# lms-org/trajectory_controller

Hardware: AMD Instinct MI355X
Metric: MPC QP solves/sec (horizon N=20, 2 inputs) at 1/2/4/8 MI355X; max|du| vs dlib (higher is better)
Workload: dtype f64; 1 GPU; batch 262144 trajectories per GPU, N=20, 2 inputs, compact (mpcControllerTobi) form, cold start, eps 0.01, max_iter 10000; global_batch=262144, horizon=20, algo=lane_fma, parallelism=batch-sharded x1, batches_in_flight=1, gather=none (1 GPU)

## Files before the change

trajectory_controller_amd/csrc/mpc_internal.h:

```cpp
#pragma once

#include <hip/hip_runtime.h>
#include <stdint.h>

namespace tpc {

constexpr int kWave = 64;

struct Knobs {
    double eps;
    uint32_t max_iter;
    uint32_t smo_iters;
};

struct CompactArgs {
    int64_t n;
    const void *v, *dy, *dphi;
    void *front, *rear;
    int32_t* iters;
    uint32_t* flags;
    const int32_t* work_hint;
    double step, wheelbase;
    double q[2], r[2], lo[2], hi[2];
    int table_key;
// ... 7 lines not shown
    double q[2], r[2], lo[2], hi[2];
    uint64_t* out;
    uint64_t* info;
    static constexpr int32_t* iters = nullptr;
    static constexpr uint32_t* flags = nullptr;
};

struct GeneralArgs {
    int64_t n, ld;
    const void *A, *B, *C, *Q, *R, *lo, *hi, *x0, *targets;
    void *controls, *v;
    void* u0;
    int32_t* iters;
    uint32_t* flags;
    const int32_t* work_hint;
    int shift_controls;
};

struct Workspace {
    void* state;
    uint32_t* ticket;
    unsigned long long* stats;
    int64_t capacity_bytes;
    uint32_t *keys, *rank, *order;
    void* sort_temp;
    size_t sort_temp_bytes;
    hipEvent_t* ev;
    int wave_group = 0;
    int group_lanes = 0;
    int max_waves = 0;
    bool group_pair = false;
    int64_t lanex_below = -1;
    int cu_count = 0;
};

constexpr int kQueueTickets = 16;
constexpr int kQueueTicketStride = 64;
constexpr int64_t kQueueTicketBytes = (int64_t)kQueueTickets * kQueueTicketStride * 4;
constexpr int64_t kWaveQueueMaxInstances = 32768;

constexpr int kAlgoMixed = 101;
constexpr int kAlgoGeneric = 100;
constexpr int kMaxHorizon = 64;
int64_t generic_scratch_bytes(int H, int dtype, int64_t n);
hipError_t generic_compact(int dtype, int H, const CompactArgs& a, const Knobs& k, void* scratch, hipStream_t s);
hipError_t generic_general(int dtype, int I, int H, const GeneralArgs& a, const Knobs& k, void* scratch, hipStream_t s);

size_t sort_temp_bytes(int64_t n);
hipError_t order_begin(void* temp, hipStream_t s);
hipError_t presolve_merge(const uint32_t* queue, const uint32_t* queue_len, int64_t n, const void* sf, const void* sr,
                          const int32_t* si, void* f, void* r, int32_t* it, uint32_t limit, hipStream_t s);
hipError_t presolve_merge_rows(const uint32_t* queue, const uint32_t* queue_len, int64_t n, const void* su, const int32_t* si,
                               void* u, int32_t* it, int rows, int64_t ld, uint32_t limit, hipStream_t s);
const uint32_t* order_queue_len(const void* temp);
hipError_t order_finish(const uint32_t* keys, const uint32_t* rank, uint32_t* order, int64_t n, void* temp,
                        hipStream_t s);

struct RolloutStepArgs {
    int64_t n, ld, ld_out, ld_nlt;
    int I, H, step, steps;
    const void *A, *B, *C;
    void* x;
    void* targets;
    const void* controls;
    const void* new_last_targets;
    void* controls_out;
    void* states_out;
    const int32_t* iters_step;
    int32_t* iters_out;
    void* sequences_out;
    const void* disturbance;
    int64_t ld_d;
};
hipError_t launch_rollout_step(int dtype, const RolloutStepArgs& a, hipStream_t s);

struct FollowArgs {
    int64_t n, ld;
    int max_points;
    const float *px, *py, *dx, *dy, *vel;
    const int32_t* count;
// ... 23 lines not shown
```

trajectory_controller_amd/csrc/mpc_lane_inst.hip:

```cpp
#include <cstdint>

#include "mpc_lane.h"
#include "mpc_lanex.h"

#ifndef TPC_LANE_H
#error "compile with -DTPC_LANE_H=<horizon>"
#endif

namespace tpc {

namespace {

constexpr int kH = TPC_LANE_H;

template <class Tag, class Kernel>
inline int pg_grid(Kernel kernel, int block) {
    constexpr int kMaxDev = 64;
    static int cache[kMaxDev] = {0};
    int dev = 0;
    if (hipGetDevice(&dev) != hipSuccess) dev = 0;
    if (dev >= 0 && dev < kMaxDev && cache[dev] > 0) return cache[dev];
    int cus = 256, per_cu = 4;
    hipDeviceProp_t prop;
    if (hipGetDeviceProperties(&prop, dev) == hipSuccess) cus = prop.multiProcessorCount;
    if (hipOccupancyMaxActiveBlocksPerMultiprocessor(&per_cu, kernel, block, 0) != hipSuccess || per_cu < 1)
        per_cu = 1;
    if (per_cu > 4) per_cu = 4;
    if (dev >= 0 && dev < kMaxDev) cache[dev] = cus * per_cu;
    return cus * per_cu;
}
struct TagState {}; struct TagFast {}; struct TagExact {}; struct TagLanex {}; template <int I> struct TagLanexG {};

inline bool wants_state(const CompactArgs&) { return false; }
inline bool wants_state(const GeneralArgs& a) { return a.controls != nullptr || a.v != nullptr; }

template <typename T, int I, class Model, class Args>
hipError_t phase1(const Args& a, const Knobs& k, const Workspace& ws, hipStream_t s) {
    T* recs = (T*)ws.state;
    hipError_t e = hipMemsetAsync(ws.ticket, 0, sizeof(uint32_t), s);
    if (e == hipSuccess) e = hipMemsetAsync(ws.stats, 0, 3 * sizeof(unsigned long long), s);
    if (e == hipSuccess) e = order_begin(ws.sort_temp, s);
    if (e != hipSuccess) return e;
    const int cd_grid = (int)((a.n + kWave - 1) / kWave);
    if (ws.ev) (void)hipEventRecord(ws.ev[0], s);
    hipLaunchKernelGGL((lane_cd_kernel<T, I, kH, Model, Args>), dim3(cd_grid), dim3(kWave), 0, s, a, k, recs,
                       ws.keys, ws.rank, (uint32_t*)ws.sort_temp, ws.stats, wants_state(a) ? 0 : 1);
    e = hipGetLastError();
    if (e != hipSuccess) return e;
    e = order_finish(ws.keys, ws.rank, ws.order, a.n, ws.sort_temp, s);
    if (e != hipSuccess) return e;
    if (ws.ev) (void)hipEventRecord(ws.ev[1], s);
    return hipSuccess;
}
template <typename T, int I, class Model, class Args>
hipError_t phase2(const Args& a, const Knobs& k, const Workspace& ws, hipStream_t s, bool only_if_refused) {
    T* recs = (T*)ws.state;
    if (wants_state(a)) {
        const int grid_cap = pg_grid<TagState>(lane_pg_kernel<T, I, kH, Model, Args>, kWave);
        const int64_t need = (a.n + kWave - 1) / kWave;
        hipLaunchKernelGGL((lane_pg_kernel<T, I, kH, Model, Args>), dim3((unsigned)(need < grid_cap ? need : grid_cap)),
                           dim3(kWave), 0, s, a, k, (const T*)recs, (const uint32_t*)ws.order, ws.ticket, ws.stats,
                           only_if_refused ? 1 : 0);
    } else {
        constexpr int bt = kWave * FusedOcc<T, kH>::value;
        const int64_t need = (a.n + bt - 1) / bt;
        const uint32_t* queue_len = order_queue_len(ws.sort_temp);
        if constexpr (Model::kFastStop) {
            if (!only_if_refused) {
                const int fast_cap = pg_grid<TagFast>(lane_pg_fused_kernel<T, I, kH, Model, Args, true>, bt);
                hipLaunchKernelGGL((lane_pg_fused_kernel<T, I, kH, Model, Args, true>),
                                   dim3((unsigned)(need < fast_cap ? need : fast_cap)), dim3(bt), 0, s, a, k,
                                   (const T*)recs, (const uint32_t*)ws.order, ws.ticket, ws.stats, queue_len);
            }
        }
// ... 32 lines not shown
        }
    }
    if constexpr (std::is_same<Args, GeneralArgs>::value && sizeof(T) == 8 && LanexPlan<kH>::built) {
        if (a.n < lanex_below(ws, true)) {
            constexpr int ng = LanexPlan<kH>::NG;
            const int64_t need = (a.n + ng - 1) / ng;
            if (wants_state(a)) {
                const int grid_cap = pg_grid<TagLanexG<I + 2>>(lanexg_pg_kernel<T, I, kH, true>, kWave);
                hipLaunchKernelGGL((lanexg_pg_kernel<T, I, kH, true>), dim3((unsigned)(need < grid_cap ? need : grid_cap)), dim3(kWave), 0, s,
                                   a, k, (const T*)ws.state, (const uint32_t*)ws.order, ws.ticket, ws.stats, (const uint32_t*)nullptr,
                                   GroupRefillBatch<LanexPlan<kH>::G>::value);
            } else {
                const int grid_cap = pg_grid<TagLanexG<I>>(lanexg_pg_kernel<T, I, kH>, kWave);
                hipLaunchKernelGGL((lanexg_pg_kernel<T, I, kH>), dim3((unsigned)(need < grid_cap ? need : grid_cap)), dim3(kWave), 0, s, a, k,
                                   (const T*)ws.state, (const uint32_t*)ws.order, ws.ticket, ws.stats, order_queue_len(ws.sort_temp),
                                   GroupRefillBatch<LanexPlan<kH>::G>::value);
            }
            e = hipGetLastError();
            if (ws.ev) (void)hipEventRecord(ws.ev[2], s);
            return e;
        }
    }
    e = phase2<T, I, Model, Args>(a, k, ws, s, false);
    if (ws.ev) (void)hipEventRecord(ws.ev[2], s);
    return e;
}

template <typename T, int I, class Model, class Args, int SUBSET = 1>
hipError_t resolve(const Args& a, const Knobs& k, const Workspace& ws, const int32_t* select, const uint32_t* gate, hipStream_t s,
                   double lambda_from = 0.0, const uint32_t* pre_len = nullptr, uint32_t pre_limit = 0u) {
    if (a.n <= 0) return hipSuccess;
    T* recs = (T*)ws.state;
    uint32_t* queue_len = ws.ticket + 1;
    hipError_t e = hipMemsetAsync(ws.ticket, 0, 32, s);
    if (e != hipSuccess) return e;
    const int grid = (int)((a.n + kWave - 1) / kWave);
    hipLaunchKernelGGL((lane_cd_kernel<T, I, kH, Model, Args, SUBSET>), dim3(grid), dim3(kWave), 0, s, a, k, recs, ws.order,
                       (uint32_t*)nullptr, queue_len, ws.stats, 1, select, gate, (T)lambda_from, pre_len, pre_limit);
    if constexpr (std::is_same<Model, CompactModel<T>>::value && sizeof(T) == 8 && LanexPlan<kH>::built) {
        constexpr int ng = LanexPlan<kH>::NG;
        const int64_t need = (a.n + ng - 1) / ng;
        if constexpr (SUBSET == 2) {
            const int64_t solo = (int64_t)pre_limit / ng;
            hipLaunchKernelGGL((lanex_pg_kernel<T, kH, true>), dim3((unsigned)(need < solo ? need : solo)), dim3(kWave), 0, s, a, k,
                               (const T*)recs, (const uint32_t*)ws.order, ws.ticket, ws.stats, (const uint32_t*)queue_len, 1, pre_limit);
            return hipGetLastError();
        }
        const int grid_cap = pg_grid<TagLanex>(lanex_pg_kernel<T, kH>, kWave);
        hipLaunchKernelGGL((lanex_pg_kernel<T, kH>), dim3((unsigned)(need < grid_cap ? need : grid_cap)), dim3(kWave), 0, s, a, k,
                           (const T*)recs, (const uint32_t*)ws.order, ws.ticket, ws.stats, (const uint32_t*)queue_len, 1);
        return hipGetLastError();
    } else if constexpr (std::is_same<Args, GeneralArgs>::value && sizeof(T) == 8 && LanexPlan<kH>::built) {
        constexpr int ng = LanexPlan<kH>::NG;
        const int64_t need = (a.n + ng - 1) / ng;
        if constexpr (SUBSET == 2) {
            const int64_t solo = (int64_t)pre_limit / ng;
            hipLaunchKernelGGL((lanexg_pg_kernel<T, I, kH, false, true>), dim3((unsigned)(need < solo ? need : solo)), dim3(kWave), 0, s,
                               a, k, (const T*)recs, (const uint32_t*)ws.order, ws.ticket, ws.stats, (const uint32_t*)queue_len, 1, pre_limit);
            return hipGetLastError();
        }
        const int grid_cap = pg_grid<TagLanexG<I>>(lanexg_pg_kernel<T, I, kH>, kWave);
        hipLaunchKernelGGL((lanexg_pg_kernel<T, I, kH>), dim3((unsigned)(need < grid_cap ? need : grid_cap)), dim3(kWave), 0, s, a, k,
                           (const T*)recs, (const uint32_t*)ws.order, ws.ticket, ws.stats, (const uint32_t*)queue_len, 1);
        return hipGetLastError();
    } else {
    constexpr int bt = kWave * FusedOcc<T, kH>::value;
    const int64_t need = (a.n + bt - 1) / bt;
// ... 71 lines not shown
```

trajectory_controller_amd/csrc/mpc_sort.hip:

```cpp
#include "mpc_internal.h"

namespace tpc {

namespace {

constexpr int kBins = 1 << 16;

constexpr int kScanBlocks = 64, kScanThreads = 256, kPerThread = kBins / kScanBlocks / kScanThreads;

__global__ __launch_bounds__(kScanThreads) void scan_sums_kernel(const uint32_t* __restrict__ hist,
                                                                 uint32_t* __restrict__ block_sum) {
    __shared__ uint32_t part[kScanThreads / 64];
    const int t = threadIdx.x;
    const int top = kBins - 1 - (blockIdx.x * kScanThreads + t) * kPerThread;
    uint32_t sum = 0;
    for (int j = 0; j < kPerThread; ++j) sum += hist[top - j];
    for (int off = 32; off > 0; off >>= 1) sum += __shfl_down(sum, off);
    if ((t & 63) == 0) part[t >> 6] = sum;
    __syncthreads();
    if (t == 0) {
        uint32_t tot = 0;
        for (int w = 0; w < kScanThreads / 64; ++w) tot += part[w];
        block_sum[blockIdx.x] = tot;
    }
}

__global__ __launch_bounds__(kScanThreads) void scan_apply_kernel(uint32_t* __restrict__ hist,
                                                                  const uint32_t* __restrict__ block_sum) {
    __shared__ uint32_t part[kScanThreads];
    const int t = threadIdx.x;
    const int top = kBins - 1 - (blockIdx.x * kScanThreads + t) * kPerThread;
    uint32_t c[kPerThread], sum = 0;
    for (int j = 0; j < kPerThread; ++j) { c[j] = hist[top - j]; sum += c[j]; }
    part[t] = sum;
    __syncthreads();
    for (int off = 1; off < kScanThreads; off <<= 1) {
        const uint32_t add = t >= off ? part[t - off] : 0u;
        __syncthreads();
        part[t] += add;
        __syncthreads();
    }
    uint32_t base = part[t] - sum;
    for (int b = 0; b < (int)blockIdx.x; ++b) base += block_sum[b];
    for (int j = 0; j < kPerThread; ++j) {
        hist[top - j] = base;
        base += c[j];
    }
}

__global__ void scatter_kernel(const uint32_t* __restrict__ keys, const uint32_t* __restrict__ rank,
                               const uint32_t* __restrict__ base, uint32_t* __restrict__ order, int64_t n) {
    for (int64_t i = (int64_t)blockIdx.x * blockDim.x + threadIdx.x; i < n; i += (int64_t)gridDim.x * blockDim.x)
        order[base[keys[i] >> 16] + rank[i]] = (uint32_t)i;
}

}

size_t sort_temp_bytes(int64_t) { return (size_t)(kBins + kScanBlocks) * sizeof(uint32_t); }

const uint32_t* order_queue_len(const void* temp) { return (const uint32_t*)temp + 127; }

hipError_t order_begin(void* temp, hipStream_t s) {
    return hipMemsetAsync(temp, 0, (size_t)kBins * sizeof(uint32_t), s);
}

hipError_t order_finish(const uint32_t* keys, const uint32_t* rank, uint32_t* order, int64_t n, void* temp,
                        hipStream_t s) {
    uint32_t* hist = (uint32_t*)temp;
    const int block = 256;
    int64_t g = (n + block - 1) / block;
    const unsigned grid = (unsigned)(g < 2048 ? g : 2048);
    uint32_t* block_sum = hist + kBins;
    hipLaunchKernelGGL(scan_sums_kernel, dim3(kScanBlocks), dim3(kScanThreads), 0, s, (const uint32_t*)hist, block_sum);
    hipLaunchKernelGGL(scan_apply_kernel, dim3(kScanBlocks), dim3(kScanThreads), 0, s, hist, (const uint32_t*)block_sum);
    hipLaunchKernelGGL(scatter_kernel, dim3(grid), dim3(block), 0, s, keys, rank, (const uint32_t*)hist, order, n);
    return hipGetLastError();
}

template <typename T>
__global__ void presolve_merge_kernel(const uint32_t* __restrict__ queue, const uint32_t* __restrict__ queue_len,
                                      const T* __restrict__ sf, const T* __restrict__ sr, const int32_t* __restrict__ si,
                                      T* __restrict__ f, T* __restrict__ r, int32_t* __restrict__ it, uint32_t limit) {
    const uint32_t nq = *queue_len;
    if (nq > limit) return;
    for (uint32_t q = blockIdx.x * blockDim.x + threadIdx.x; q < nq; q += gridDim.x * blockDim.x) {
        const uint32_t k = queue[q];
        f[k] = sf[k];
        r[k] = sr[k];
        if (it) it[k] = si[k];
    }
}
__global__ void presolve_merge_rows_kernel(const uint32_t* __restrict__ queue, const uint32_t* __restrict__ queue_len,
                                           const double* __restrict__ su, const int32_t* __restrict__ si, double* __restrict__ u,
                                           int32_t* __restrict__ it, int rows, int64_t ld, uint32_t limit) {
    const uint32_t nq = *queue_len;
    if (nq > limit) return;
    for (uint32_t q = blockIdx.x * blockDim.x + threadIdx.x; q < nq; q += gridDim.x * blockDim.x) {
        const uint32_t k = queue[q];
        for (int j = 0; j < rows; ++j) u[(int64_t)j * ld + k] = su[(int64_t)j * ld + k];
        if (it) it[k] = si[k];
    }
}
hipError_t presolve_merge_rows(const uint32_t* queue, const uint32_t* queue_len, int64_t n, const void* su, const int32_t* si,
                               void* u, int32_t* it, int rows, int64_t ld, uint32_t limit, hipStream_t s) {
    const int64_t blocks = (n + 255) / 256;
    hipLaunchKernelGGL(presolve_merge_rows_kernel, dim3((unsigned)(blocks < 256 ? blocks : 256)), dim3(256), 0, s, queue, queue_len,
                       (const double*)su, si, (double*)u, it, rows, ld, limit);
    return hipGetLastError();
// ... 11 lines not shown
```

trajectory_controller_amd/csrc/mpc_ub_inst.hip:

```cpp
#include <cstdint>
#include <type_traits>

#include "mpc_ub.h"

#ifndef TPC_UB_H
#error "compile with -DTPC_UB_H=<horizon>"
#endif

namespace tpc {

hipError_t ub_pg_asm_launch(const CompactArgs& a, const Knobs& k, const Workspace& ws, int64_t need, hipStream_t s);
hipError_t ub_pg_asm_launch_h10(const CompactArgs& a, const Knobs& k, const Workspace& ws, int64_t need, hipStream_t s);

namespace {

constexpr int kH = TPC_UB_H;

template <class Tag, class Kernel>
inline int ub_grid(Kernel kernel, int block) {
    constexpr int kMaxDev = 64;
    static int cache[kMaxDev] = {0};
    int dev = 0;
    if (hipGetDevice(&dev) != hipSuccess) dev = 0;
    if (dev >= 0 && dev < kMaxDev && cache[dev] > 0) return cache[dev];
    int cus = 256, per_cu = 4;
    hipDeviceProp_t prop;
    if (hipGetDeviceProperties(&prop, dev) == hipSuccess) cus = prop.multiProcessorCount;
    if (hipOccupancyMaxActiveBlocksPerMultiprocessor(&per_cu, kernel, block, 0) != hipSuccess || per_cu < 1)
        per_cu = 1;
    if (per_cu > 4) per_cu = 4;
    if (dev >= 0 && dev < kMaxDev) cache[dev] = cus * per_cu;
    return cus * per_cu;
}
template <typename T, bool EQB, int MODE> struct TagPg {};

template <typename T, bool EQB>
hipError_t phase1(const CompactArgs& a, const Knobs& k, const Workspace& ws, hipStream_t s) {
    T* recs = (T*)ws.state;
    hipError_t e = hipMemsetAsync(ws.ticket, 0, sizeof(uint32_t), s);
    if (e == hipSuccess) e = hipMemsetAsync(ws.stats, 0, 3 * sizeof(unsigned long long), s);
    if (e == hipSuccess) e = order_begin(ws.sort_temp, s);
    if (e != hipSuccess) return e;
    const int cd_grid = (int)((a.n + kWave - 1) / kWave);
    if (ws.ev) (void)hipEventRecord(ws.ev[0], s);
    hipLaunchKernelGGL((ub_cd_kernel<T, kH, EQB>), dim3(cd_grid), dim3(kWave), 0, s, a, k, recs, ws.keys, ws.rank,
                       (uint32_t*)ws.sort_temp, ws.stats);
    e = hipGetLastError();
    if (e != hipSuccess) return e;
    e = order_finish(ws.keys, ws.rank, ws.order, a.n, ws.sort_temp, s);
    if (e != hipSuccess) return e;
    if (ws.ev) (void)hipEventRecord(ws.ev[1], s);
    return hipSuccess;
}
template <typename T, bool EQB, int MODE>
hipError_t pg_launch(const CompactArgs& a, const Knobs& k, const Workspace& ws, hipStream_t s) {
    constexpr int bt = kWave * UbPlan<T, kH>::occ;
    const int64_t need = (a.n + bt - 1) / bt;
#if (TPC_UB_H == 20 || TPC_UB_H == 10) && !defined(TPC_UB_NO_ASM)
    if constexpr (sizeof(T) == 8 && EQB && MODE == 2) {
        const int64_t waves = (a.n + kWave - 1) / kWave;
        return kH == 20 ? ub_pg_asm_launch(a, k, ws, waves, s) : ub_pg_asm_launch_h10(a, k, ws, waves, s);
    }
#endif
    int cap = ub_grid<TagPg<T, EQB, MODE>>(ub_pg_kernel<T, kH, EQB, MODE>, bt);
    if (ws.max_waves > 0) {
        const int lim = ws.max_waves / UbPlan<T, kH>::occ > 1 ? ws.max_waves / UbPlan<T, kH>::occ : 1;
        if (cap > lim) cap = lim;
    }
    hipLaunchKernelGGL((ub_pg_kernel<T, kH, EQB, MODE>), dim3((unsigned)(need < cap ? need : cap)), dim3(bt), 0, s, a, k,
                       (const T*)ws.state, (const uint32_t*)ws.order, ws.ticket, ws.stats, order_queue_len(ws.sort_temp));
    return hipGetLastError();
}

template <typename T, bool EQB>
// ... 40 lines not shown
```

trajectory_controller_amd/csrc/tpc_mpc_api.cpp:

```cpp
#include "tpc_mpc_context.h"
#include "tpc_mpc_experimental.h"
#include "auto_table.h"
#include "mpc_queue_key_table.h"
#include "mpc_grad_model.h"
#include "mpc_polish_model.h"
#include "mpc_rollout_newton.h"
#include "mpc_newton_compact.h"
#include "mpc_compact_grad.h"
#include "mpc_tangent_model.h"

#include <cmath>
#include <cstdlib>
#include <mutex>
#include <vector>

namespace tpc {
#define TPC_DECL_H(h)                                                                             \
    hipError_t lane_compact_h##h(int, const CompactArgs&, const Knobs&, const Workspace&, hipStream_t); \
    hipError_t lane_general_h##h(int, int, const GeneralArgs&, const Knobs&, const Workspace&, hipStream_t); \
    hipError_t lane_resolve_compact_h##h(const CompactArgs&, const Knobs&, const Workspace&, const int32_t*, const uint32_t*, hipStream_t, double, const uint32_t*, uint32_t); \
    hipError_t lane_presolve_compact_h##h(const CompactArgs&, const Knobs&, const Workspace&, double, uint32_t, hipStream_t); \
    hipError_t lane_resolve_general_h##h(int, const GeneralArgs&, const Knobs&, const Workspace&, const int32_t*, const uint32_t*, hipStream_t, double, const uint32_t*, uint32_t); \
    hipError_t lane_presolve_general_h##h(int, const GeneralArgs&, const Knobs&, const Workspace&, double, uint32_t, hipStream_t); \
    hipError_t wave_compact_h##h(int, const CompactArgs&, const Knobs&, const Workspace&, hipStream_t); \
// ... 274 lines not shown
    ws->ticket = h->ws_words;
    ws->stats = (unsigned long long*)(h->ws_words + 4);
    ws->capacity_bytes = 0;
    ws->ev = h->profiling ? h->ev : nullptr;
    ws->wave_group = h->opt_wave_group;
    ws->group_lanes = group_lanes(h, H, dtype, n, form);
    ws->max_waves = h->max_waves;
    if (h->pre_busy && h->pre_group_waves > 0 && (ws->max_waves == 0 || ws->max_waves > h->pre_group_waves))
        ws->max_waves = h->pre_group_waves;
    ws->group_pair = group_pair(h, H, dtype, n, form);
    ws->lanex_below = h->opt_lanex_below;
    ws->cu_count = h->cu_count;
    h->ev_valid = h->profiling;
    h->last_algo = algo;
    ws->keys = ws->rank = ws->order = nullptr;
    ws->sort_temp = nullptr;
    ws->sort_temp_bytes = 0;
    if (algo == kAlgoGeneric) {
        int rc = ensure(h, &h->ws_state, &h->ws_bytes, pad256(generic_scratch_bytes(H, dtype, n)));
        if (rc) return rc;
        ws->state = h->ws_state;
        ws->capacity_bytes = h->ws_bytes;
    }
    if (algo == TPC_MPC_ALGO_WAVE) {
        int rc = ensure(h, &h->ws_state, &h->ws_bytes, pad256(n * 4) + kQueueTicketBytes);
        if (rc) return rc;
        ws->order = (uint32_t*)h->ws_state;
        ws->ticket = (uint32_t*)((char*)h->ws_state + pad256(n * 4));
        ws->capacity_bytes = h->ws_bytes;
    }
    if (algo == TPC_MPC_ALGO_LANE || algo == TPC_MPC_ALGO_LANE_FMA || algo == TPC_MPC_ALGO_GROUP) {
        const int64_t rec_b = pad256(lane_rec_len(H, dtype) * (int64_t)esize(dtype) * n);
        const int64_t col_b = pad256(n * 4);
        const size_t tmp_b = sort_temp_bytes(n);
        int rc = ensure(h, &h->ws_state, &h->ws_bytes, rec_b + 3 * col_b + pad256((int64_t)tmp_b));
        if (rc) return rc;
        char* b = (char*)h->ws_state;
        ws->state = b;
        ws->keys = (uint32_t*)(b + rec_b);
        ws->rank = (uint32_t*)(b + rec_b + col_b);
        ws->order = (uint32_t*)(b + rec_b + 2 * col_b);
        ws->sort_temp = b + rec_b + 3 * col_b;
        ws->sort_temp_bytes = tmp_b;
        ws->capacity_bytes = h->ws_bytes;
    }
    return TPC_MPC_OK;
}

int resolve_reserve(tpc_mpc_context* h, int H, int dtype, int64_t n) { return reserve_lane_workspace(h, H, dtype, n); }
int resolve_workspace(tpc_mpc_context* h, int H, int dtype, int64_t n, Workspace* ws) {
    const bool ev_valid = h->ev_valid;
    const int last_algo = h->last_algo;
    const int rc = prepare_workspace(h, TPC_MPC_ALGO_LANE, H, dtype, n, ws);
    h->ev_valid = ev_valid;
    h->last_algo = last_algo;
    ws->ev = nullptr;
    ws->ticket = h->ws_words + 16;
    ws->stats = (unsigned long long*)(h->ws_words + 18);
    return rc;
}

hipError_t copy_rows(void* dst, int64_t dpitch, const void* src, int64_t spitch, int64_t width, int64_t rows,
                     hipMemcpyKind kind, hipStream_t s) {
    if (rows <= 0 || width <= 0) return hipSuccess;
    if (dpitch == width && spitch == width) return hipMemcpyAsync(dst, src, (size_t)(width * rows), kind, s);
    return hipMemcpy2DAsync(dst, (size_t)dpitch, src, (size_t)spitch, (size_t)width, (size_t)rows, kind, s);
}

int check_general_io(tpc_mpc_context* h, const tpc_mpc_general_io* io, int mem) {
    if (!io) return fail(h, TPC_MPC_ERR_BAD_ARG, "null io");
    if (io->inputs != 1 && io->inputs != 2) return fail(h, TPC_MPC_ERR_BAD_ARG, "inputs must be 1 or 2");
    if (io->n < 0 || io->ld < io->n || io->n > 0x7fffffffll)
        return fail(h, TPC_MPC_ERR_BAD_ARG, "need 0 <= n <= ld, n < 2^31");
    if (mem != TPC_MPC_HOST && mem != TPC_MPC_DEVICE) return fail(h, TPC_MPC_ERR_BAD_ARG, "bad memory kind");
    return TPC_MPC_OK;
}

int check_model(tpc_mpc_context* h, const tpc_mpc_general_io* io, bool also = true) {
    if (!io->A || !io->B || !io->C || !io->Q || !io->R || !io->lower || !io->upper || !io->x0 || !io->targets || !also)
        return fail(h, TPC_MPC_ERR_BAD_ARG, "null batch pointer");
    return TPC_MPC_OK;
}
int check_polish(tpc_mpc_context* h, const tpc_mpc_polish* q) {
    if (!q) return fail(h, TPC_MPC_ERR_BAD_ARG, "null polish struct");
    if (!(q->tol > 0.0) || q->max_rounds < 0)
        return fail(h, TPC_MPC_ERR_BAD_ARG, "polish needs tol > 0 and max_rounds >= 0");
    return TPC_MPC_OK;
}
int check_steps(tpc_mpc_context* h, int32_t steps) {
// ... 53 lines not shown
int stream_order_end(tpc_mpc_context* h, hipStream_t s) {
    HIP_TRY(h, hipEventRecord(h->done_ev, s));
    h->last_stream = s;
    h->have_last = true;
    return TPC_MPC_OK;
}

int finish_flags(tpc_mpc_context* h, uint32_t* flags_out, hipStream_t s) {
    if (!flags_out) return TPC_MPC_OK;
    uint32_t f = 0;
    HIP_TRY(h, hipMemcpyAsync(&f, h->ws_words + 1, sizeof(f), hipMemcpyDeviceToHost, s));
    HIP_TRY(h, hipStreamSynchronize(s));
    *flags_out = f;
    return TPC_MPC_OK;
}

int reserve_lane_workspace(tpc_mpc_context* h, int H, int dtype, int64_t n) {
    const bool ev_valid = h->ev_valid;
    const int last_algo = h->last_algo;
    Workspace ws;
    const int rc = prepare_workspace(h, horizon_specialised(H) ? TPC_MPC_ALGO_LANE : kAlgoGeneric, H, dtype, n, &ws);
    h->ev_valid = ev_valid;
    h->last_algo = last_algo;
    return rc;
}

int context_new(int device, int cu_count, tpc_mpc_context** out) {
    tpc_mpc_context* h = new (std::nothrow) tpc_mpc_context;
    if (!h) return fail(nullptr, TPC_MPC_ERR_ALLOC, "out of host memory");
    h->device = device;
    h->cu_count = cu_count;
    h->device_cu_count = cu_count;
    hipError_t e = hipSetDevice(device);
    if (e == hipSuccess) e = hipMalloc((void**)&h->ws_words, 128);
    if (e == hipSuccess) e = hipMemset(h->ws_words, 0, 128);
    if (e == hipSuccess) e = hipHostMalloc(&h->pin_host, 512, hipHostMallocMapped | hipHostMallocCoherent);
    if (e == hipSuccess) e = hipHostGetDevicePointer(&h->pin_dev, h->pin_host, 0);
    if (e == hipSuccess) e = hipEventCreateWithFlags(&h->done_ev, hipEventDisableTiming);
    if (e != hipSuccess) {
        (void)tpc_mpc_destroy(h);
        return fail(nullptr, TPC_MPC_ERR_HIP, "create: %s", hipGetErrorString(e));
    }
    std::memset(h->pin_host, 0, 512);
    *out = h;
    return TPC_MPC_OK;
}

static double presolve_lambda(const tpc_mpc_params* p);
static int presolve_scratch(tpc_mpc_context* h, int H, int dtype, int64_t n, int64_t side_bytes, Workspace* ws, char** side) {
    const int64_t rec_b = pad256(lane_rec_len(H, dtype) * (int64_t)esize(dtype) * n), col_b = pad256(n * 4);
    const size_t tmp_b = sort_temp_bytes(n);
    const int64_t lane_b = rec_b + 3 * col_b + pad256((int64_t)tmp_b);
    int rc = ensure(h, &h->pre, &h->pre_bytes, lane_b + side_bytes);
    if (rc) return rc;
    if (!h->pre_stream) HIP_TRY(h, hipStreamCreateWithFlags(&h->pre_stream, hipStreamNonBlocking));
    if (!h->pre_fork) HIP_TRY(h, hipEventCreateWithFlags(&h->pre_fork, hipEventDisableTiming));
    if (!h->pre_done) HIP_TRY(h, hipEventCreateWithFlags(&h->pre_done, hipEventDisableTiming));
    char* b = (char*)h->pre;
    std::memset(ws, 0, sizeof(*ws));
    ws->state = b;
    ws->keys = (uint32_t*)(b + rec_b);
    ws->rank = (uint32_t*)(b + rec_b + col_b);
    ws->order = (uint32_t*)(b + rec_b + 2 * col_b);
    ws->sort_temp = b + rec_b + 3 * col_b;
    ws->sort_temp_bytes = tmp_b;
    ws->capacity_bytes = lane_b;
    ws->ev = nullptr;
    ws->lanex_below = h->opt_lanex_below;
    ws->cu_count = h->cu_count;
    ws->ticket = h->ws_words + 24;
    ws->stats = (unsigned long long*)(h->ws_words + 26);
    *side = b + lane_b;
    return TPC_MPC_OK;
}
static bool presolve_share(tpc_mpc_context* h, int64_t n, Presolve* ps) {
    const int simds = (h->device_cu_count > 0 ? h->device_cu_count : 256) * 4;
    const int solo_waves = simds * 7 / 16;
    if (n > (int64_t)solo_waves * 8 * 5) return false;
    ps->limit = (uint32_t)solo_waves * 8u;
    ps->group_waves = simds - solo_waves;
    return true;
}

int general_launch(tpc_mpc_context* h, const tpc_mpc_params* p, const tpc_mpc_general_io* io, hipStream_t s) {
    const int I = io->inputs, H = p->horizon;
    const int64_t n = io->n;
    const int algo = pick_algo(h, p->algo, I, H, n, p->dtype, fma_general_usable(H, io->controls_inout, io->v_inout), false,
                                   group_general_usable(p->dtype, H, io->controls_inout, io->v_inout));
    if (algo < 0) return fail(h, TPC_MPC_ERR_BAD_HORIZON, "the WAVE kernel exists for the specialised horizons with inputs*horizon <= 64 only; use LANE or AUTO");
    GeneralArgs a;
    std::memset(&a, 0, sizeof(a));
    a.n = n; a.ld = io->ld; a.shift_controls = 1;
    a.A = io->A; a.B = io->B; a.C = io->C; a.Q = io->Q; a.R = io->R; a.lo = io->lower; a.hi = io->upper;
    a.x0 = io->x0; a.targets = io->targets; a.controls = io->controls_inout; a.v = io->v_inout;
    a.u0 = io->u0; a.iters = io->iters;
    a.flags = h->ws_words + 1;
    a.work_hint = take_hint(h, n);
    const bool fix = wants_cap_resolve(p, algo) && !a.controls && !a.v;
    int rc = TPC_MPC_OK;
    if (fix && !a.iters) rc = cap_iters_buffer(h, n, &a.iters);
    if (!rc && fix) rc = resolve_reserve(h, H, p->dtype, n);
    if (rc) return rc;
    Presolve ps;
    const double lf = presolve_lambda(p);
// ... 142 lines not shown
    hipError_t e = resolve_compact(p->horizon, a, knobs_of(p), ws2, s, ps->lambda_from, ps->queue_len, ps->limit);
    if (e != hipSuccess) return hip_fail(h, e, "kernel launch");
    return TPC_MPC_OK;
}

static bool queue_key_table_applies(const tpc_mpc_params* p, int algo) {
    return algo == TPC_MPC_ALGO_LANE_FMA && p->dtype == TPC_MPC_F64 && p->horizon == kQueueKeyH &&
           p->weight_y == kQueueKeyWeights[0] && p->weight_phi == kQueueKeyWeights[1] &&
           p->weight_steering_front == kQueueKeyWeights[2] && p->weight_steering_rear == kQueueKeyWeights[3] &&
           p->step_size == kQueueKeyStep && p->wheelbase == kQueueKeyWheelbase &&
           p->lower[0] == kQueueKeyLower && p->lower[1] == kQueueKeyLower &&
           p->upper[0] == kQueueKeyUpper && p->upper[1] == kQueueKeyUpper && p->eps == kQueueKeyEps &&
           p->max_iter == kQueueKeyMaxIter && p->smo_iters == kQueueKeySmoIters;
}

int compact_launch_ps(tpc_mpc_context* h, const tpc_mpc_params* p, int64_t n, const void* v, const void* dy,
                      const void* dphi, void* front, void* rear, int32_t* iters, hipStream_t s, Presolve* ps) {
    const int algo = pick_algo(h, p->algo, 2, p->horizon, n, p->dtype, fma_usable(p));
    if (algo < 0) return fail(h, TPC_MPC_ERR_BAD_HORIZON, "the WAVE kernel exists for the specialised horizons with inputs*horizon <= 64 only; use LANE or AUTO");
    CompactArgs a;
    compact_args(h, p, n, v, dy, dphi, front, rear, iters, &a);
    a.work_hint = take_hint(h, n);
    a.table_key = h->opt_queue_key && queue_key_table_applies(p, algo) ? 1 : 0;
    h->last_queue_key = a.work_hint ? kQueueKeyHint : (a.table_key ? kQueueKeyTableUsed : kQueueKeyLambda);
    const bool fix = wants_cap_resolve(p, algo) && a.flags;
    int rc = TPC_MPC_OK;
    if (fix && !a.iters) rc = cap_iters_buffer(h, n, &a.iters);
    if (!rc && fix) rc = resolve_reserve(h, p->horizon, p->dtype, n);
    if (rc) return rc;
    ps->select = a.iters;
    Workspace ws;
    rc = prepare_workspace(h, algo, p->horizon, p->dtype, n, &ws);
    if (rc) return rc;
    hipError_t e = dispatch_compact(algo, p->horizon, p->dtype, a, knobs_of(p), ws, s);
    if (e != hipSuccess) return hip_fail(h, e, "kernel launch");
    if (ps->deferred) return TPC_MPC_OK;
    return presolve_finish(h, p, n, v, dy, dphi, front, rear, iters, s, ps);
}

int compact_launch(tpc_mpc_context* h, const tpc_mpc_params* p, int64_t n, const void* v, const void* dy,
                   const void* dphi, void* front, void* rear, int32_t* iters, hipStream_t s) {
    Presolve ps;
    int rc = presolve_begin(h, p, n, v, dy, dphi, s, &ps);
    if (!rc) rc = compact_launch_ps(h, p, n, v, dy, dphi, front, rear, iters, s, &ps);
    if (rc && ps.on) {
        h->pre_busy = false;
        (void)hipEventRecord(h->pre_done, h->pre_stream);
        (void)hipStreamWaitEvent(s, h->pre_done, 0);
    }
    return rc;
}

}

namespace {

struct StagedExtra {
    const int64_t* src_ld = nullptr;
    const int64_t* dst_ld = nullptr;
    const int* width = nullptr;
    int inout = -1;
};

template <int NIn, int NOut, class Run>
int staged_run(tpc_mpc_context* h, const tpc_mpc_general_io* io, int mem, void* stream, uint32_t* flags_out,
               int64_t ws_bytes, const void* const (&src)[NIn], void* const (&dst)[NOut],
               const int64_t (&rows)[NIn + NOut], Run run, const StagedExtra& x = StagedExtra()) {
    const int64_t n = io->n;
    if (h->host_only) {
        uint32_t f = 0;
        (void)run(io->ld, src, dst, (hipStream_t) nullptr, &f);
        if (flags_out) *flags_out = f;
        return TPC_MPC_OK;
    }
    HIP_TRY(h, hipSetDevice(h->device));
    hipStream_t s = (hipStream_t)stream;
    StreamOrderScope order(h, s);
    int rc = order.begin();
    if (rc) return rc;
    rc = ensure(h, &h->grad_ws, &h->grad_ws_bytes, pad256(ws_bytes));
    if (rc) return rc;
    const int64_t lds = (n + 63) / 64 * 64;
    const void* sin[NIn];
    void* sout[NOut];
    for (int c = 0; c < NIn; ++c) sin[c] = src[c];
    for (int c = 0; c < NOut; ++c) sout[c] = dst[c];
    int64_t ld = io->ld;
    const bool host = mem == TPC_MPC_HOST;
// ... 166 lines not shown
            *out = h;
            return TPC_MPC_OK;
        }
        int count = 0;
        hipError_t e = hipGetDeviceCount(&count);
        if (e != hipSuccess || count <= 0)
            return fail(nullptr, TPC_MPC_ERR_NO_DEVICE, "no HIP device: %s",
                        e != hipSuccess ? hipGetErrorString(e) : "count == 0");
        if (device < 0 || device >= count) return fail(nullptr, TPC_MPC_ERR_NO_DEVICE, "device index out of range");
        hipDeviceProp_t prop;
        e = hipGetDeviceProperties(&prop, device);
        if (e != hipSuccess) return fail(nullptr, TPC_MPC_ERR_NO_DEVICE, "%s", hipGetErrorString(e));
        if (std::strncmp(prop.gcnArchName, "gfx950", 6) != 0)
            return fail(nullptr, TPC_MPC_ERR_NO_DEVICE, "device is %s, this library carries gfx950 code only",
                        prop.gcnArchName);
        return context_new(device, prop.multiProcessorCount, out);
    });
}

int tpc_mpc_destroy(tpc_mpc_handle h) {
    if (!h) return TPC_MPC_OK;
    return guarded(nullptr, [&]() -> int {
        if (h->host_only) { delete h; return TPC_MPC_OK; }
        (void)hipSetDevice(h->device);
        one_shot_destroy(h);
        comm_destroy(h);
        for (int i = 0; i < tpc_mpc_context::kMaxKids; ++i) {
            if (h->kid_stream[i]) { (void)hipStreamSynchronize(h->kid_stream[i]); (void)hipStreamDestroy(h->kid_stream[i]); }
            if (h->kid_done[i]) (void)hipEventDestroy(h->kid_done[i]);
            if (h->kids[i]) (void)tpc_mpc_destroy(h->kids[i]);
        }
        if (h->fork_ev) (void)hipEventDestroy(h->fork_ev);
        if (h->ws_state) (void)hipFree(h->ws_state);
        if (h->ws_words) (void)hipFree(h->ws_words);
        if (h->stage) (void)hipFree(h->stage);
        if (h->roll) (void)hipFree(h->roll);
        if (h->cap_iters) (void)hipFree(h->cap_iters);
        if (h->grad_ws) (void)hipFree(h->grad_ws);
        if (h->newton) (void)hipFree(h->newton);
        if (h->newton_fb) (void)hipFree(h->newton_fb);
        if (h->mix) (void)hipFree(h->mix);
        if (h->gather) (void)hipFree(h->gather);
        if (h->pre_stream) { (void)hipStreamSynchronize(h->pre_stream); (void)hipStreamDestroy(h->pre_stream); }
        if (h->pre_fork) (void)hipEventDestroy(h->pre_fork);
        if (h->pre_done) (void)hipEventDestroy(h->pre_done);
        if (h->pre) (void)hipFree(h->pre);
        if (h->hint_own) (void)hipFree(h->hint_own);
        if (h->pin_host) (void)hipHostFree(h->pin_host);
        if (h->done_ev) (void)hipEventDestroy(h->done_ev);
        for (auto& e : h->ev) if (e) (void)hipEventDestroy(e);
        delete h;
        return TPC_MPC_OK;
    });
}

const char* tpc_mpc_last_error(tpc_mpc_handle h) { return h ? h->err : g_create_error; }

int tpc_mpc_solve_batch_compact(tpc_mpc_handle h, const tpc_mpc_params* p, int64_t n, const void* v,
                                const void* delta_y, const void* delta_phi, void* steering_front,
                                void* steering_rear, int32_t* iters, uint32_t* flags_out, int mem,
                                void* stream) {
    return guarded(h, [&]() -> int {
        int rc = check_common(h, p);
        if (rc) return rc;
        rc = check_compact_model(h, p);
        if (rc) return rc;
        if (n < 0 || n > 0x7fffffffll) return fail(h, TPC_MPC_ERR_BAD_ARG, "need 0 <= n < 2^31");
        if (mem != TPC_MPC_HOST && mem != TPC_MPC_DEVICE) return fail(h, TPC_MPC_ERR_BAD_ARG, "bad memory kind");
        if (n == 0) { if (flags_out) *flags_out = 0; return TPC_MPC_OK; }
        if (!v || !delta_y || !delta_phi || !steering_front || !steering_rear)
            return fail(h, TPC_MPC_ERR_BAD_ARG, "null batch pointer");
        HIP_TRY(h, hipSetDevice(h->device));
        hipStream_t s = (hipStream_t)stream;
        const int64_t es = (int64_t)esize(p->dtype);
        StreamOrderScope order(h, s);
        rc = order.begin();
        if (rc) return rc;
        HIP_TRY(h, hipMemsetAsync(h->ws_words + 1, 0, sizeof(uint32_t), s));
        if (mem == TPC_MPC_DEVICE) {
            rc = compact_launch(h, p, n, v, delta_y, delta_phi, steering_front, steering_rear, iters, s);
            if (rc) return rc;
        } else {
            const int64_t col = pad256(n * es), icol = pad256(n * 4);
            rc = ensure(h, &h->stage, &h->stage_bytes, 5 * col + icol);
            if (rc) return rc;
            char* b = (char*)h->stage;
            HIP_TRY(h, hipMemcpyAsync(b, v, n * es, hipMemcpyHostToDevice, s));
            HIP_TRY(h, hipMemcpyAsync(b + col, delta_y, n * es, hipMemcpyHostToDevice, s));
            HIP_TRY(h, hipMemcpyAsync(b + 2 * col, delta_phi, n * es, hipMemcpyHostToDevice, s));
            int32_t* d_it = iters ? (int32_t*)(b + 5 * col) : nullptr;
            rc = compact_launch(h, p, n, b, b + col, b + 2 * col, b + 3 * col, b + 4 * col, d_it, s);
            if (rc) return rc;
            HIP_TRY(h, hipMemcpyAsync(steering_front, b + 3 * col, n * es, hipMemcpyDeviceToHost, s));
            HIP_TRY(h, hipMemcpyAsync(steering_rear, b + 4 * col, n * es, hipMemcpyDeviceToHost, s));
            if (iters) HIP_TRY(h, hipMemcpyAsync(iters, d_it, n * 4, hipMemcpyDeviceToHost, s));
            HIP_TRY(h, hipStreamSynchronize(s));
        }
        rc = order.end();
        if (rc) return rc;
        return finish_flags(h, flags_out, s);
    });
}

int tpc_mpc_solve_one(tpc_mpc_handle h, const tpc_mpc_params* p, double v, double delta_y,
                      double delta_phi, double* steering_front, double* steering_rear) {
    return guarded(h, [&]() -> int {
        if (!h) return fail(nullptr, TPC_MPC_ERR_BAD_ARG, "null handle");
        if (!steering_front || !steering_rear) return fail(h, TPC_MPC_ERR_BAD_ARG, "null output pointer");
        int rc = check_common(h, p, true);
        if (rc) return rc;
        rc = check_compact_model(h, p);
// ... 1538 lines not shown
```

trajectory_controller_amd/csrc/tpc_mpc_context.h:

```cpp
#pragma once

#include "../../include/tpc_mpc.h"

#include <hip/hip_runtime.h>

#include <cstdarg>
#include <cstdio>
#include <cstring>
#include <exception>
#include <new>

#include "mpc_internal.h"

namespace tpc {
struct OneShot;
int context_new(int device, int cu_count, tpc_mpc_context** out);
struct Comm;
}

constexpr size_t kTpcErrLen = 512;

struct tpc_mpc_context {
    int device = 0;
    int cu_count = 0;
    int device_cu_count = 0;
    char err[kTpcErrLen] = "";
    void* ws_state = nullptr;
    int64_t ws_bytes = 0;
    uint32_t* ws_words = nullptr;
    void* stage = nullptr;
    int64_t stage_bytes = 0;
    void* roll = nullptr;
    int64_t roll_bytes = 0;
    void* cap_iters = nullptr;
    int64_t cap_iters_bytes = 0;
    void* grad_ws = nullptr;
    int64_t grad_ws_bytes = 0;
    void* newton = nullptr;
    int64_t newton_bytes = 0;
    void* newton_fb = nullptr;
    int64_t newton_fb_bytes = 0;
    void* pre = nullptr;
    int64_t pre_bytes = 0;
    hipStream_t pre_stream = nullptr;
    hipEvent_t pre_fork = nullptr, pre_done = nullptr;
    bool pre_busy = false;
    int pre_group_waves = 0;
    void* mix = nullptr;
    int64_t mix_bytes = 0;
    void* pin_host = nullptr;
    void* pin_dev = nullptr;
    tpc::OneShot* one = nullptr;
    const int32_t* hint = nullptr;
    int64_t hint_n = 0;
    void* hint_own = nullptr;
    int64_t hint_own_bytes = 0;
    bool opt_queue_key = true;
    int last_queue_key = 0;
    bool collect_flags = true;
    uint32_t one_flags = 0;
    int32_t one_iters = 0;
    bool one_valid = false;
// ... 129 lines not shown
```

Measured before the change: 61.12 million solves/s.

## Merge per-solve memsets into one reset and fuse radix scan kernels

Places the sort histogram and the ticket/stats words in one persistent contiguous device region, so a single memset at solve entry replaces the separate ticket, stats and histogram memsets in phase1 and resolve. Also fuses the two-kernel scan (block sums, then apply) into one kernel where each block re-reads all bins above it as uint4 and writes offsets into a separate output array. This cuts launch and memset count per solve but adds redundant histogram reads in the later scan blocks, and depends on correct reset_armed bookkeeping across code paths.

New measurement: 61.29 million solves/s, median of 6. No clear change (+0.3%).

```diff
diff --git a/trajectory_controller_amd/csrc/mpc_internal.h b/trajectory_controller_amd/csrc/mpc_internal.h
--- a/trajectory_controller_amd/csrc/mpc_internal.h
+++ b/trajectory_controller_amd/csrc/mpc_internal.h
@@ -63,6 +63,7 @@
     bool group_pair = false;
     int64_t lanex_below = -1;
     int cu_count = 0;
+    bool reset_done = false;
 };
 
 constexpr int kQueueTickets = 16;
@@ -77,6 +78,8 @@
 hipError_t generic_compact(int dtype, int H, const CompactArgs& a, const Knobs& k, void* scratch, hipStream_t s);
 hipError_t generic_general(int dtype, int I, int H, const GeneralArgs& a, const Knobs& k, void* scratch, hipStream_t s);
 
+constexpr int kSortBins = 1 << 16;
+constexpr int kSortGapWords = 128;
 size_t sort_temp_bytes(int64_t n);
 hipError_t order_begin(void* temp, hipStream_t s);
 hipError_t presolve_merge(const uint32_t* queue, const uint32_t* queue_len, int64_t n, const void* sf, const void* sr,
diff --git a/trajectory_controller_amd/csrc/mpc_lane_inst.hip b/trajectory_controller_amd/csrc/mpc_lane_inst.hip
--- a/trajectory_controller_amd/csrc/mpc_lane_inst.hip
+++ b/trajectory_controller_amd/csrc/mpc_lane_inst.hip
@@ -37,9 +37,12 @@
 template <typename T, int I, class Model, class Args>
 hipError_t phase1(const Args& a, const Knobs& k, const Workspace& ws, hipStream_t s) {
     T* recs = (T*)ws.state;
-    hipError_t e = hipMemsetAsync(ws.ticket, 0, sizeof(uint32_t), s);
-    if (e == hipSuccess) e = hipMemsetAsync(ws.stats, 0, 3 * sizeof(unsigned long long), s);
-    if (e == hipSuccess) e = order_begin(ws.sort_temp, s);
+    hipError_t e = hipSuccess;
+    if (!ws.reset_done) {
+        e = hipMemsetAsync(ws.ticket, 0, sizeof(uint32_t), s);
+        if (e == hipSuccess) e = hipMemsetAsync(ws.stats, 0, 3 * sizeof(unsigned long long), s);
+        if (e == hipSuccess) e = order_begin(ws.sort_temp, s);
+    }
     if (e != hipSuccess) return e;
     const int cd_grid = (int)((a.n + kWave - 1) / kWave);
     if (ws.ev) (void)hipEventRecord(ws.ev[0], s);
@@ -138,7 +141,7 @@
     if (a.n <= 0) return hipSuccess;
     T* recs = (T*)ws.state;
     uint32_t* queue_len = ws.ticket + 1;
-    hipError_t e = hipMemsetAsync(ws.ticket, 0, 32, s);
+    hipError_t e = ws.reset_done ? hipSuccess : hipMemsetAsync(ws.ticket, 0, 32, s);
     if (e != hipSuccess) return e;
     const int grid = (int)((a.n + kWave - 1) / kWave);
     hipLaunchKernelGGL((lane_cd_kernel<T, I, kH, Model, Args, SUBSET>), dim3(grid), dim3(kWave), 0, s, a, k, recs, ws.order,
diff --git a/trajectory_controller_amd/csrc/mpc_sort.hip b/trajectory_controller_amd/csrc/mpc_sort.hip
--- a/trajectory_controller_amd/csrc/mpc_sort.hip
+++ b/trajectory_controller_amd/csrc/mpc_sort.hip
@@ -4,32 +4,27 @@
 
 namespace {
 
-constexpr int kBins = 1 << 16;
+constexpr int kBins = kSortBins;
+constexpr int kBaseAt = kSortBins + kSortGapWords;
 
 constexpr int kScanBlocks = 64, kScanThreads = 256, kPerThread = kBins / kScanBlocks / kScanThreads;
 
-__global__ __launch_bounds__(kScanThreads) void scan_sums_kernel(const uint32_t* __restrict__ hist,
-                                                                 uint32_t* __restrict__ block_sum) {
-    __shared__ uint32_t part[kScanThreads / 64];
+__global__ __launch_bounds__(kScanThreads) void scan_kernel(const uint32_t* __restrict__ hist, uint32_t* __restrict__ first) {
+    __shared__ uint32_t part[kScanThreads];
+    __shared__ uint32_t above_part[kScanThreads / 64];
     const int t = threadIdx.x;
-    const int top = kBins - 1 - (blockIdx.x * kScanThreads + t) * kPerThread;
-    uint32_t sum = 0;
-    for (int j = 0; j < kPerThread; ++j) sum += hist[top - j];
-    for (int off = 32; off > 0; off >>= 1) sum += __shfl_down(sum, off);
-    if ((t & 63) == 0) part[t >> 6] = sum;
-    __syncthreads();
-    if (t == 0) {
-        uint32_t tot = 0;
-        for (int w = 0; w < kScanThreads / 64; ++w) tot += part[w];
-        block_sum[blockIdx.x] = tot;
+    const int own = kBins - (int)blockIdx.x * kScanThreads * kPerThread;
+    static_assert(kPerThread == 4, "the bins above are read as uint4, one block's worth of them per trip");
+    const uint4* above4 = reinterpret_cast<const uint4*>(hist + own);
+    uint32_t above = 0;
+#pragma unroll 8
+    for (int i = 0; i < (int)blockIdx.x; ++i) {
+        const uint4 q = above4[i * kScanThreads + t];
+        above += q.x + q.y + q.z + q.w;
     }
-}
-
-__global__ __launch_bounds__(kScanThreads) void scan_apply_kernel(uint32_t* __restrict__ hist,
-                                                                  const uint32_t* __restrict__ block_sum) {
-    __shared__ uint32_t part[kScanThreads];
-    const int t = threadIdx.x;
-    const int top = kBins - 1 - (blockIdx.x * kScanThreads + t) * kPerThread;
+    for (int off = 32; off > 0; off >>= 1) above += __shfl_down(above, off);
+    if ((t & 63) == 0) above_part[t >> 6] = above;
+    const int top = own - 1 - t * kPerThread;
     uint32_t c[kPerThread], sum = 0;
     for (int j = 0; j < kPerThread; ++j) { c[j] = hist[top - j]; sum += c[j]; }
     part[t] = sum;
@@ -41,9 +36,9 @@
         __syncthreads();
     }
     uint32_t base = part[t] - sum;
-    for (int b = 0; b < (int)blockIdx.x; ++b) base += block_sum[b];
+    for (int w = 0; w < kScanThreads / 64; ++w) base += above_part[w];
     for (int j = 0; j < kPerThread; ++j) {
-        hist[top - j] = base;
+        first[top - j] = base;
         base += c[j];
     }
 }
@@ -56,9 +51,9 @@
 
 }
 
-size_t sort_temp_bytes(int64_t) { return (size_t)(kBins + kScanBlocks) * sizeof(uint32_t); }
+size_t sort_temp_bytes(int64_t) { return (size_t)(kBaseAt + kBins) * sizeof(uint32_t); }
 
-const uint32_t* order_queue_len(const void* temp) { return (const uint32_t*)temp + 127; }
+const uint32_t* order_queue_len(const void* temp) { return (const uint32_t*)temp + kBaseAt + 127; }
 
 hipError_t order_begin(void* temp, hipStream_t s) {
     return hipMemsetAsync(temp, 0, (size_t)kBins * sizeof(uint32_t), s);
@@ -70,10 +65,9 @@
     const int block = 256;
     int64_t g = (n + block - 1) / block;
     const unsigned grid = (unsigned)(g < 2048 ? g : 2048);
-    uint32_t* block_sum = hist + kBins;
-    hipLaunchKernelGGL(scan_sums_kernel, dim3(kScanBlocks), dim3(kScanThreads), 0, s, (const uint32_t*)hist, block_sum);
-    hipLaunchKernelGGL(scan_apply_kernel, dim3(kScanBlocks), dim3(kScanThreads), 0, s, hist, (const uint32_t*)block_sum);
-    hipLaunchKernelGGL(scatter_kernel, dim3(grid), dim3(block), 0, s, keys, rank, (const uint32_t*)hist, order, n);
+    uint32_t* first = hist + kBaseAt;
+    hipLaunchKernelGGL(scan_kernel, dim3(kScanBlocks), dim3(kScanThreads), 0, s, (const uint32_t*)hist, first);
+    hipLaunchKernelGGL(scatter_kernel, dim3(grid), dim3(block), 0, s, keys, rank, (const uint32_t*)first, order, n);
     return hipGetLastError();
 }
 
diff --git a/trajectory_controller_amd/csrc/mpc_ub_inst.hip b/trajectory_controller_amd/csrc/mpc_ub_inst.hip
--- a/trajectory_controller_amd/csrc/mpc_ub_inst.hip
+++ b/trajectory_controller_amd/csrc/mpc_ub_inst.hip
@@ -37,9 +37,12 @@
 template <typename T, bool EQB>
 hipError_t phase1(const CompactArgs& a, const Knobs& k, const Workspace& ws, hipStream_t s) {
     T* recs = (T*)ws.state;
-    hipError_t e = hipMemsetAsync(ws.ticket, 0, sizeof(uint32_t), s);
-    if (e == hipSuccess) e = hipMemsetAsync(ws.stats, 0, 3 * sizeof(unsigned long long), s);
-    if (e == hipSuccess) e = order_begin(ws.sort_temp, s);
+    hipError_t e = hipSuccess;
+    if (!ws.reset_done) {
+        e = hipMemsetAsync(ws.ticket, 0, sizeof(uint32_t), s);
+        if (e == hipSuccess) e = hipMemsetAsync(ws.stats, 0, 3 * sizeof(unsigned long long), s);
+        if (e == hipSuccess) e = order_begin(ws.sort_temp, s);
+    }
     if (e != hipSuccess) return e;
     const int cd_grid = (int)((a.n + kWave - 1) / kWave);
     if (ws.ev) (void)hipEventRecord(ws.ev[0], s);
diff --git a/trajectory_controller_amd/csrc/tpc_mpc_api.cpp b/trajectory_controller_amd/csrc/tpc_mpc_api.cpp
--- a/trajectory_controller_amd/csrc/tpc_mpc_api.cpp
+++ b/trajectory_controller_amd/csrc/tpc_mpc_api.cpp
@@ -330,16 +330,15 @@
     if (algo == TPC_MPC_ALGO_LANE || algo == TPC_MPC_ALGO_LANE_FMA || algo == TPC_MPC_ALGO_GROUP) {
         const int64_t rec_b = pad256(lane_rec_len(H, dtype) * (int64_t)esize(dtype) * n);
         const int64_t col_b = pad256(n * 4);
-        const size_t tmp_b = sort_temp_bytes(n);
-        int rc = ensure(h, &h->ws_state, &h->ws_bytes, rec_b + 3 * col_b + pad256((int64_t)tmp_b));
+        int rc = ensure(h, &h->ws_state, &h->ws_bytes, rec_b + 3 * col_b);
         if (rc) return rc;
         char* b = (char*)h->ws_state;
         ws->state = b;
         ws->keys = (uint32_t*)(b + rec_b);
         ws->rank = (uint32_t*)(b + rec_b + col_b);
         ws->order = (uint32_t*)(b + rec_b + 2 * col_b);
-        ws->sort_temp = b + rec_b + 3 * col_b;
-        ws->sort_temp_bytes = tmp_b;
+        ws->sort_temp = h->sort_region;
+        ws->sort_temp_bytes = sort_temp_bytes(n);
         ws->capacity_bytes = h->ws_bytes;
     }
     return TPC_MPC_OK;
@@ -353,6 +352,7 @@
     h->ev_valid = ev_valid;
     h->last_algo = last_algo;
     ws->ev = nullptr;
+    ws->reset_done = h->reset_armed;
     ws->ticket = h->ws_words + 16;
     ws->stats = (unsigned long long*)(h->ws_words + 18);
     return rc;
@@ -472,8 +472,9 @@
     h->cu_count = cu_count;
     h->device_cu_count = cu_count;
     hipError_t e = hipSetDevice(device);
-    if (e == hipSuccess) e = hipMalloc((void**)&h->ws_words, 128);
-    if (e == hipSuccess) e = hipMemset(h->ws_words, 0, 128);
+    if (e == hipSuccess) e = hipMalloc(&h->sort_region, sort_temp_bytes(0));
+    if (e == hipSuccess) e = hipMemset(h->sort_region, 0, sort_temp_bytes(0));
+    if (e == hipSuccess) h->ws_words = (uint32_t*)h->sort_region + kSortBins;
     if (e == hipSuccess) e = hipHostMalloc(&h->pin_host, 512, hipHostMallocMapped | hipHostMallocCoherent);
     if (e == hipSuccess) e = hipHostGetDevicePointer(&h->pin_dev, h->pin_host, 0);
     if (e == hipSuccess) e = hipEventCreateWithFlags(&h->done_ev, hipEventDisableTiming);
@@ -508,8 +509,8 @@
     ws->ev = nullptr;
     ws->lanex_below = h->opt_lanex_below;
     ws->cu_count = h->cu_count;
-    ws->ticket = h->ws_words + 24;
-    ws->stats = (unsigned long long*)(h->ws_words + 26);
+    ws->ticket = h->ws_words + 64;
+    ws->stats = (unsigned long long*)(h->ws_words + 66);
     *side = b + lane_b;
     return TPC_MPC_OK;
 }
@@ -718,6 +719,7 @@
     Workspace ws;
     rc = prepare_workspace(h, algo, p->horizon, p->dtype, n, &ws);
     if (rc) return rc;
+    ws.reset_done = h->reset_armed;
     hipError_t e = dispatch_compact(algo, p->horizon, p->dtype, a, knobs_of(p), ws, s);
     if (e != hipSuccess) return hip_fail(h, e, "kernel launch");
     if (ps->deferred) return TPC_MPC_OK;
@@ -740,6 +742,22 @@
 }
 
 namespace {
+
+struct ResetScope {
+    tpc_mpc_context* h;
+    explicit ResetScope(tpc_mpc_context* hh) : h(hh) {}
+    int begin(const tpc_mpc_params* p, int64_t n, hipStream_t s) {
+        const int algo = pick_algo(h, p->algo, 2, p->horizon, n, p->dtype, fma_usable(p));
+        if (algo == TPC_MPC_ALGO_LANE || algo == TPC_MPC_ALGO_LANE_FMA || algo == TPC_MPC_ALGO_GROUP) {
+            HIP_TRY(h, hipMemsetAsync(h->sort_region, 0, (size_t)(kSortBins + 64) * sizeof(uint32_t), s));
+            h->reset_armed = true;
+        } else {
+            HIP_TRY(h, hipMemsetAsync(h->ws_words + 1, 0, sizeof(uint32_t), s));
+        }
+        return TPC_MPC_OK;
+    }
+    ~ResetScope() { h->reset_armed = false; }
+};
 
 struct StagedExtra {
     const int64_t* src_ld = nullptr;
@@ -972,7 +990,7 @@
         }
         if (h->fork_ev) (void)hipEventDestroy(h->fork_ev);
         if (h->ws_state) (void)hipFree(h->ws_state);
-        if (h->ws_words) (void)hipFree(h->ws_words);
+        if (h->sort_region) (void)hipFree(h->sort_region);
         if (h->stage) (void)hipFree(h->stage);
         if (h->roll) (void)hipFree(h->roll);
         if (h->cap_iters) (void)hipFree(h->cap_iters);
@@ -1016,7 +1034,9 @@
         StreamOrderScope order(h, s);
         rc = order.begin();
         if (rc) return rc;
-        HIP_TRY(h, hipMemsetAsync(h->ws_words + 1, 0, sizeof(uint32_t), s));
+        ResetScope reset(h);
+        rc = reset.begin(p, n, s);
+        if (rc) return rc;
         if (mem == TPC_MPC_DEVICE) {
             rc = compact_launch(h, p, n, v, delta_y, delta_phi, steering_front, steering_rear, iters, s);
             if (rc) return rc;
diff --git a/trajectory_controller_amd/csrc/tpc_mpc_context.h b/trajectory_controller_amd/csrc/tpc_mpc_context.h
--- a/trajectory_controller_amd/csrc/tpc_mpc_context.h
+++ b/trajectory_controller_amd/csrc/tpc_mpc_context.h
@@ -28,6 +28,8 @@
     void* ws_state = nullptr;
     int64_t ws_bytes = 0;
     uint32_t* ws_words = nullptr;
+    void* sort_region = nullptr;
+    bool reset_armed = false;
     void* stage = nullptr;
     int64_t stage_bytes = 0;
     void* roll = nullptr;
```
